# istellartech/GELATO

Hardware: AMD Instinct MI355X
Metric: residual+Jacobian evals/sec (and ms/eval), 6-phase x 64-node LGR mesh (higher is better)
Workload: dtype f64

## Files before the change

gelato_amd/csrc/gel_eval_kernel.h:

```cpp
#pragma once

namespace gel {

enum ParkSlot { PK_Q0 = 0, PK_Q1, PK_Q2, PK_Q3, PK_V0, PK_V1, PK_V2, PK_DJJ, PK_LV0, PK_LV1, PK_LV2,
                PK_FP0, PK_FP1, PK_FP2, PK_FP3, PK_FP4, PK_FP5, PK_FP6, PK_FP7, PK_COUNT };
constexpr int kStageLd = 17;
constexpr int kWaveLds = PK_COUNT * 64;
static_assert(kWaveLds >= 64 * kStageLd, "the MFMA staging tile must fit the wave's park region");
constexpr int kCoopStageOff = PK_LV0 * 64;
static_assert(kWaveLds - kCoopStageOff >= 64 * 11, "the cooperative hand-over area must fit behind the early park slots");
constexpr int kXldsPipeFrom = kLongPhaseFrom;
constexpr int kSlabRowsMax = 68, kPackRows = 36, kParkRes = (PK_LV2 + 1) * 64;
constexpr int kPipeSlabK = 8;
constexpr int wave_lds_doubles(bool jac, bool mfma, bool pack, bool split = false, bool longp = true) {
  return jac ? kWaveLds : (!mfma ? kParkRes : (split ? 64 * kStageLd  : (pack ? kParkRes + 4 * 64  : (longp ? 2 * 4 * kPipeSlabK * 11 + 64 * kPipeSlabK  : kSlabRowsMax * 11))));
}
static_assert(wave_lds_doubles(false, true, false, true) >= kParkRes, "residual-only split form: park over the result tile");
static_assert(wave_lds_doubles(false, true, true) >= 64 * 11 && wave_lds_doubles(false, true, false) >= 64 * 11 && wave_lds_doubles(false, true, false, false, false) >= 64 * 11, "hand-over area");
static_assert(wave_lds_doubles(false, true, true) >= kParkRes && wave_lds_doubles(false, true, false) >= kParkRes && wave_lds_doubles(false, true, false, false, false) >= kParkRes, "residual-only park");

constexpr int kSlotPT = 0, kSlotVM = 3, kSlotVP = 6;

#ifndef GEL_MIN_WAVES_PER_SIMD
#define GEL_MIN_WAVES_PER_SIMD 4
// ... 875 lines not shown
      PosCentreTail pt;
      double cen_rho = 0.0, cen_P = 0.0, cen_inv_a = 0.0;
      double dir2 = 0.0;
      EarthHalf aeh{1.0, 0.0};
      bool have_aeh = false;
#ifndef GEL_AEH
#define GEL_AEH aeh
#endif
#ifndef GEL_X_NOPOS
#define GEL_X_NOPOS 0
#endif
#ifndef GEL_X_NOQUAT
#define GEL_X_NOQUAT 0
#endif
#ifndef GEL_X_NOVEL
#define GEL_X_NOVEL 0
#endif
      const bool aero_on = AERO && akinds != 0;
      const bool a_need_alpha = AERO && (akinds & 5) != 0;
#define GEL_AERO_NEED_EA(ip_, wn_, we_)                                                                                \
  do {                                                                                                                 \
    if (!have_aeh && __builtin_amdgcn_ballot_w64(wind_needs_angle(ip_, wn_, we_)) != 0) {                               \
      int jl_ = jc;                                                                                                    \
      asm volatile("" : "+v"(jl_));    \
      const double tau_ = P.tau[ph.toff + jl_];                                                                        \
      const EarthAngle e_ = earth_angle((tau_ * (tf - to) / 2 + (tf + to) / 2) * P.ut);                                \
      aeh.ch = e_.ch; aeh.sh = e_.sh; have_aeh = true;                                                                 \
    }                                                                                                                  \
  } while (0)
#define GEL_AERO_FETCH()                                                                                               \
  const int ab_[3] = {load_const(&aph->base[0]), load_const(&aph->base[1]), load_const(&aph->base[2])};                \
  const double ax_[3] = {load_const(&aph->ilx[0]), load_const(&aph->ilx[1]), load_const(&aph->ilx[2])};                \
  const int n8_ = 8 * n, j08_ = 8 * j0
#define GEL_AERO_ENTRY(blk, col, a_, nv2_, d_, ind_, rho_, okl_, a_cc, a_ac, a_qc, a_isc, a_ok)                         \
  do {                                                                                                                 \
    double t_ = 0.0, dq_ = 0.0, qp_ = 0.0;                                                                             \
    const double ac_ = a_ac;                                                                                           \
    {                                                                                                                  \
      const double qc_ = a_qc;                                                                                         \
      qp_ = 0.5 * (rho_) * (nv2_);                                                                                     \
      dq_ = qp_ - qc_;                                                                                                 \
      if (a_need_alpha) {                                                                                              \
        const double cp_ = aero_cos(a_, nv2_, d_, ind_);                                                               \
        const bool okd_ = aero_dalpha(cp_, nv2_, a_cc, a_isc, a_ok, t_);                                               \
        if (__builtin_amdgcn_ballot_w64(!okd_) != 0) {                                                                 \
          const double t2_ = aero_acos(cp_, nv2_) - ac_;                                                               \
          t_ = okd_ ? t_ : t2_;                                                                                        \
        }                                                                                                              \
      }                                                                                                                \
    }                                                                                                                  \
    _Pragma("unroll") for (int kind = 0; kind < 3; kind++) {                                                           \
      if ((blk) == 2 && kind == 1) continue;                             \
      const double df_ = (kind == 0) ? t_ : ((kind == 1) ? dq_ : qp_ * t_ + dq_ * ac_);                                \
      const double gv = -(df_ * ax_[kind]);                                                                            \
      if (okl_) AEMIT(ab_[kind] + (((blk) == 0 ? 1 : ((blk) == 1 ? 4 : 7)) + (col)) * n8_ + j08_, gv);                 \
    }                                                                                                                  \
  } while (0)
#if GEL_CA_CACHE
      Bracket ca_br = no_bracket();
#define GEL_CA_BRACKET (JAC ? &ca_br : (Bracket*)nullptr)
#else
#define GEL_CA_BRACKET nullptr
#endif
      struct ParkSink { lds_double* park; GEL_DEV void put(int i, double v) const { if (!(AERO && (i == PCS_P || i == PCS_IH))) park[(PK_FP0 + i) * 64] = v; } };
      constexpr int PK_ACC = PK_FP0 + PCS_P, PK_AAC = PK_FP0 + PCS_IH, PK_AQC = PK_LV2;
      static_assert(PCS_COUNT == 8 && PK_FP7 == PK_FP0 + 7, "PosCentre's early members fill FP0-7");
      {
        PosPart pp;
        double v[3], w[3], F[3], dir[3];
        const double r[3] = {fresh_product(re[0], P.up), fresh_product(re[1], P.up), fresh_product(re[2], P.up)};
        if (JAC) pp = pos_part<true, ParkSink>(r, tb, P.barC20, nullptr, ParkSink{park}, &pt);
        else pp = pos_part(r, tb, P.barC20);
        const bool cen_windy = AERO && __builtin_amdgcn_ballot_w64(!(pp.wn == 0.0 && pp.we == 0.0)) != 0;
        if (__builtin_amdgcn_ballot_w64(wind_needs_angle(pp.inv_p, pp.wn, pp.we)) != 0) {
          const EarthAngle e0 = earth_angle(tn);
          eh.ch = e0.ch; eh.sh = e0.sh; have_eh = true;
          if (aero_on) PARK_SET(PK_ACC, tn);
        }
        EarthAngle ea{1.0, 0.0, 1.0, 0.0};
        if (have_eh) ea = full_angle(eh);
        wind_eci_or_calm(r, ea, pp.shp, pp.chp, pp.inv_p, pp.wn, pp.we, w);
#pragma unroll
        for (int c = 0; c < 3; c++) v[c] = PARK_GET(PK_V0 + c) * P.uv;
        aero_force(r, v, pp.rho, pp.inv_a, w, ph.area, tb, F, GEL_CA_BRACKET);
#define GEL_T (ph.thrust - ph.nozzle * pp.P)
#define GEL_TDC(name) const double name[3] = {GEL_T * dir[0], GEL_T * dir[1], GEL_T * dir[2]}
        {
          const double q[4] = {PARK_GET(PK_Q0), PARK_GET(PK_Q1), PARK_GET(PK_Q2), PARK_GET(PK_Q3)};
          thrust_dir(q, dir);
        }
        double tm[3];
        {
          GEL_TDC(Tdc);
          accel_parts(Tdc, F, inv_m, pp.g, inv_uv, tm, fc);
        }
        if (rb) {
#ifndef GEL_RES_XPOSE_VEL_AIR
#define GEL_RES_XPOSE_VEL_AIR 1
#endif
          if (!JAC || GEL_RES_XPOSE_VEL_AIR) {
            double cv[3];
#pragma unroll
            for (int c = 0; c < 3; c++) cv[c] = PARK_GET(PK_LV0 + c) - fc[c] * (tf - to) * hT;
            RSTORE_ROWS(wave_lds + PK_LV0 * 64, 3, rs_v, cv);
          } else {
#pragma unroll
            for (int c = 0; c < 3; c++) {
              const double cv = PARK_GET(PK_LV0 + c) - fc[c] * (tf - to) * hT;
              RSTORE(rs_v + 3 * gn + c, cv);
              GEL_CHK(cv);
            }
          }
        }
        if (JAC) {
          asm volatile("" ::: "memory");
          PARK_SET(PK_LV0, pp.shp); PARK_SET(PK_LV1, pp.chp);
          if (!AERO) PARK_SET(PK_LV2, pp.inv_p);
        }
        if (JAC && lead && !P.fd_recompute) GEL_MASS_CLOSED(tm);
        if (JAC && ph.air_fd && (SPLIT && P.split_vel ? !lead : lead)) {
          double f[3];
          {
            const double djj = PARK_GET(PK_DJJ);
#pragma unroll
            for (int k = 0; k < 3; k++) {
              if (SPLIT && P.split_vel && k != part - 1) continue;
              double vp[3], Fp[3];
#pragma unroll
              for (int c = 0; c < 3; c++) vp[c] = ((k == c) ? (PARK_GET(PK_V0 + c) + dx) : PARK_GET(PK_V0 + c)) * P.uv;
              const double r[3] = {fresh_product(re[0], P.up), fresh_product(re[1], P.up), fresh_product(re[2], P.up)};
              aero_force(r, vp, pp.rho, pp.inv_a, w, ph.area, tb, Fp, GEL_CA_BRACKET);
              GEL_TDC(Tdc);
              accel(Tdc, Fp, inv_m, pp.g, inv_uv, f);
#pragma unroll
              for (int c = 0; c < 3; c++) EMIT(ph.s_vv + 3 * k + c, ((c == k) ? djj : 0.0) + FDQ(f[c], fc[c]));
            }
          }
        }
        if (JAC && lead) {
          double f[3];
          if (!P.fd_recompute) {
            GEL_QUAT_CLOSED(GEL_T);
          } else if (P.fd_recompute) {
            const double q[4] = {PARK_GET(PK_Q0), PARK_GET(PK_Q1), PARK_GET(PK_Q2), PARK_GET(PK_Q3)};
#pragma unroll 1
            for (int k = 0; k < 4; k++) {
              double qp[4];
#pragma unroll
              for (int c = 0; c < 4; c++) qp[c] = (k == c) ? (q[c] + dx) : q[c];
              double dp[3];
              thrust_dir(qp, dp);
              const double Td[3] = {GEL_T * dp[0], GEL_T * dp[1], GEL_T * dp[2]};
              accel(Td, F, inv_m, pp.g, inv_uv, f);
#pragma unroll
              for (int c = 0; c < 3; c++) EMIT(ph.s_vq + 3 * k + c, FDQ(f[c], fc[c]));
            }
            GEL_TDC(Tdc);
            accel(Tdc, F, frcp((me + dx) * P.um), pp.g, inv_uv, f);
#pragma unroll
            for (int c = 0; c < 3; c++) EMIT(kSlotVM + c, FDQ(f[c], fc[c]));
          }
          if (!ph.t_fd) {
            const double vt[3] = {fc[0] * hT, fc[1] * hT, fc[2] * hT};
            EMIT_GROUP(3, ph.s_vt, vt, CG_VT, 0, true, true);
          }
        }
        if (aero_on) {
          asm volatile("" ::: "memory");
          const double ra[3] = {fresh_product(re[0], P.up), fresh_product(re[1], P.up), fresh_product(re[2], P.up)};
          double va[3], wa[3], a0[3];
#pragma unroll
          for (int c = 0; c < 3; c++) va[c] = PARK_GET(PK_V0 + c) * P.uv;
          if (have_eh) {
            const EarthAngle e1 = earth_angle(PARK_GET(PK_ACC) * P.ut);
            aeh.ch = e1.ch; aeh.sh = e1.sh; have_aeh = true;
          }
          if (cen_windy) {
            PosCentre pcx;
            double wn_, we_, p_, ip_, ih_;
            pos_centre_tail(pt, pp.rho, pp.P, tb, pcx, wn_, we_);
            geodetic_p_ih(ra[0], ra[1], ra[2], p_, ip_, ih_);
            EarthAngle e2{1.0, 0.0, 1.0, 0.0};
            if (have_aeh) e2 = full_angle(GEL_AEH);
            wind_eci(ra, e2, PARK_GET(PK_LV0), PARK_GET(PK_LV1), ip_, wn_, we_, wa);
          } else {
            wa[0] = 0.0; wa[1] = 0.0; wa[2] = 0.0;
          }
          const double nv2 = aero_vair2(ra, va, wa, a0);
          const double ind = frsqrt(fmax(dir[0] * dir[0] + dir[1] * dir[1] + dir[2] * dir[2], 1.0e-300));
          const double cc = a_need_alpha ? aero_cos(a0, nv2, dir, ind) : 0.0;
          const double alpha_c = a_need_alpha ? aero_acos(cc, nv2) : 0.0;
          const double qdyn_c = 0.5 * pp.rho * nv2;
          double sc, isc;
          fsqrt_rsqrt(fmax((1.0 - cc) * (1.0 + cc), 1.0e-300), sc, isc);
          const bool centre_ok = (cc <= 1.0) && (nv2 >= 1.0e-12) && (sc > 1.0e-6);
          GEL_AERO_FETCH();
          const double ail_[3] = {load_const(&aph->il[0]), load_const(&aph->il[1]), load_const(&aph->il[2])};
#pragma unroll
          for (int kind = 0; kind < 3; kind++) {
            const double il = ail_[kind];
            const double cv = 1.0 - ((kind == 0) ? alpha_c : (kind == 1) ? qdyn_c : qdyn_c * alpha_c) * il;
            AEMIT(ab_[kind] + j08_, cv);
            GEL_CHK(cv);
          }
          if (a_need_alpha && !GEL_X_NOQUAT) {
            const double q[4] = {PARK_GET(PK_Q0), PARK_GET(PK_Q1), PARK_GET(PK_Q2), PARK_GET(PK_Q3)};
#pragma unroll
            for (int c = 0; c < 4; c++) {
              double qp[4], dp[3];
#pragma unroll
              for (int d = 0; d < 4; d++) qp[d] = (d == c) ? q[d] + dx : q[d];
              thrust_dir(qp, dp);
              const double indp = frsqrt(fmax(dp[0] * dp[0] + dp[1] * dp[1] + dp[2] * dp[2], 1.0e-300));
              GEL_AERO_ENTRY(2, c, a0, nv2, dp, indp, pp.rho, true, cc, alpha_c, qdyn_c, isc, centre_ok);
              __builtin_amdgcn_sched_barrier(0);
            }
          }
#pragma unroll
          for (int c = 0; c < (GEL_X_NOVEL ? 0 : 3); c++) {
            double vp[3], a[3];
#pragma unroll
            for (int d = 0; d < 3; d++) vp[d] = ((d == c) ? PARK_GET(PK_V0 + d) + dx : PARK_GET(PK_V0 + d)) * P.uv;
            const double nv2p = aero_vair2(ra, vp, wa, a);
            GEL_AERO_ENTRY(1, c, a, nv2p, dir, ind, pp.rho, true, cc, alpha_c, qdyn_c, isc, centre_ok);
            __builtin_amdgcn_sched_barrier(0);
          }
          PARK_SET(PK_ACC, cc); PARK_SET(PK_AAC, centre_ok ? alpha_c : -alpha_c); PARK_SET(PK_AQC, qdyn_c);
        }
        if (JAC) {
          asm volatile("" ::: "memory");
          PARK_SET(PK_Q0, fc[0]); PARK_SET(PK_Q1, fc[1]); PARK_SET(PK_Q2, fc[2]); PARK_SET(PK_Q3, dir[0]); PARK_SET(PK_DJJ, dir[1]);
          dir2 = dir[2];
          cen_rho = pp.rho; cen_P = pp.P; cen_inv_a = pp.inv_a;
        }
#undef GEL_TDC
#undef GEL_T
      }
      if (JAC && (!SPLIT || part)) {
        const int k0 = SPLIT ? part - 1 : 0, k1 = SPLIT ? part : 3;
#define GEL_POS_SWEEP_F(rp, pq, f_)                                                                           \
  do {                                                                                                        \
    double wq_[3], Fp_[3];                                                                                    \
    GEL_NEED_EARTH_ANGLE((pq).inv_p, (pq).wn, (pq).we);                                                       \
    EarthAngle ea{1.0, 0.0, 1.0, 0.0};                                                                        \
    if (have_eh) ea = full_angle(eh);                                                                         \
    wind_eci_or_calm(rp, ea, (pq).shp, (pq).chp, (pq).inv_p, (pq).wn, (pq).we, wq_);                          \
    const double vq_[3] = {PARK_GET(PK_V0) * P.uv, PARK_GET(PK_V1) * P.uv, PARK_GET(PK_V2) * P.uv};           \
    aero_force(rp, vq_, (pq).rho, (pq).inv_a, wq_, ph.area, tb, Fp_, GEL_CA_BRACKET);                         \
    const double Tp_ = ph.thrust - ph.nozzle * (pq).P;                                                        \
// ... 247 lines not shown
```

gelato_amd/csrc/gel_host.hip:

```cpp
#include <hip/hip_runtime.h>

#include <algorithm>
#include <cmath>
#include <cstdio>
#include <chrono>
#include <atomic>
#include <cstdlib>
#include <cstring>
#include <memory>
#include <string>
#include <thread>
#include <vector>

#include "gel_host_handle.h"

namespace gelhost {
namespace {
thread_local std::string g_err;
}
int fail(int code, const std::string& msg) {
  g_err = msg;
  return code;
}
}
// ... 1256 lines not shown
  for (int k = 0; k < 3; k++) {
    const size_t n = p->aero.rows[k].size();
    off_c[k] = atotal; atotal += (io->aero_con[k] && n) ? n : 0;
    off_j[k] = atotal; atotal += (io->aero_con[k] && n && io->aero_jac[k]) ? aero_jac_len(p, k) : 0;
    aero = aero || (io->aero_con[k] && n);
  }
  const size_t nrows_out = rows ? R + 7 * nfn : 0;
  if (rows || aero) HIPCHK(p->h_arena.reserve(nrows_out + atotal));
  double* const h_rows = p->h_arena.get();
  double* const h_aero = h_rows + nrows_out;
  const bool x_pinned = p->cb_x[0].get() && (x == p->cb_x[0].get() || x == p->cb_x[1].get());
  if (!x_pinned) std::memcpy(p->h_x.get(), x, (size_t)p->dims.num_vars * 8);
  const double* const xin = x_pinned ? x : p->h_x.get();
  gel::ProblemDev dv = p->dev;
  dv.flag = p->h_flag.get();
  const bool want_jac = io->vals_full != nullptr;
  const bool fused = io->res || want_jac;
  static const int cb_mode = [] { const char* e = getenv("GEL_CB_MODE"); return e ? atoi(e) : 0; }();
  const bool split_exact = p->exact && want_jac;
  bool aero_jac = false;
  for (int k = 0; k < 3; k++) aero_jac = aero_jac || (io->aero_con[k] && io->aero_jac[k] && !p->aero.rows[k].empty());
  const bool split_aero = p->exact_aero && aero_jac;
  const bool split_rows = p->exact_rows && rows && io->rows_jfn;
  const bool coo = want_jac && cb_mode != 3 && !p->exact && !split_aero && !split_rows && coo_direct(p);
  if (coo) {
    if ((rc = ensure_full(p))) return rc;
    dv.coo_full = p->h_full.get(); dv.coo = p->d_coo.get();
  }
  dv.split_vel = 1;
  const bool own_res = io->res && p->cb_res.get() && io->res == p->cb_res.get();
  double* const res_to = own_res ? p->cb_res.get() : p->h_res.get();
  gel::AeroLaunchOut out;
  if (aero)
    for (int k = 0; k < 3; k++) {
      const size_t n = p->aero.rows[k].size();
      out.nrows[k] = (int32_t)n;
      out.con[k] = (io->aero_con[k] && n) ? h_aero + off_c[k] : nullptr;
      out.jac[k] = (out.con[k] && io->aero_jac[k]) ? h_aero + off_j[k] : nullptr;
    }
  if (cb_mode == 3 || !fused || split_exact || split_aero || split_rows) {
    if (fused) HIPCHK(launch_defects(p, dv, 1, xin, res_to, want_jac ? p->h_jv.get() : nullptr, p->stream.get()));
    if (rows) HIPCHK(launch_rows_kinds(p, dv, 1, xin, h_rows, io->rows_jfn ? h_rows + R : nullptr, p->stream.get()));
    if (aero) HIPCHK(launch_aero_kinds(p, dv, (int)p->aero.nodes.size(), p->aero.d_nodes.get(), 1, xin, out, p->stream.get()));
  } else {
    arm_done(p, dv);
    HIPCHK(gel::launch_callback(dv, want_jac, xin, res_to, want_jac ? p->h_jv.get() : nullptr,
                                aero ? (int)p->aero.nodes.size() : 0, p->aero.d_nodes.get(), aero ? &out : nullptr,
                                (int)nlin, p->d_lin_rows.get(), (int)nfn, p->d_fn_rows.get(), rows ? h_rows : nullptr,
                                (rows && io->rows_jfn) ? h_rows + R : nullptr, p->stream.get()));
  }
  HIPCHK(wait_done(p, dv));
  if (io->res && !own_res) std::memcpy(io->res, p->h_res.get(), (size_t)11 * p->dims.N * 8);
  if (want_jac) {
    if (coo) finish_full(p, io->vals_full, io->fill_constants);
    else scatter_full(p, p->h_jv.get(), io->vals_full, io->fill_constants);
  }
  if (rows) {
    std::memcpy(io->rows_con, h_rows, R * 8);
    if (io->rows_jfn) std::memcpy(io->rows_jfn, h_rows + R, 7 * nfn * 8);
  }
  if (aero)
    for (int k = 0; k < 3; k++) {
      if (out.con[k]) std::memcpy(io->aero_con[k], out.con[k], p->aero.rows[k].size() * 8);
      if (out.jac[k]) std::memcpy(io->aero_jac[k], out.jac[k], aero_jac_len(p, k) * 8);
    }
  if (*p->h_flag.get()) { *p->h_flag.get() = 0; return GEL_NONFINITE; }
  return GEL_OK;
}

int gel_table_limits(int32_t wind_rows, int32_t ca_rows, int32_t n, int64_t* info) {
  if (wind_rows < 2 || ca_rows < 2 || !info) return fail(GEL_ERR_ARG, "bad argument");
  const size_t T = gel::staged_table_doubles(wind_rows, ca_rows), Tp = gel::padded_table_doubles(wind_rows, ca_rows);
  info[0] = (int64_t)T;
  info[1] = (int64_t)lds_room(gel::eval_lds_bytes_max(wind_rows, ca_rows) / 8 - Tp, true);
  info[2] = (int64_t)lds_room(gel::aero_lds_bytes(wind_rows, ca_rows) / 8 - Tp, true);
  info[3] = (n >= 2 && n < gel::kMeshMaxThreads) ? (int64_t)lds_room(gel::mesh_vector_doubles(n), true) : -1;
  info[4] = (int64_t)lds_room(gel::table_lds_bytes(wind_rows, ca_rows) / 8 - T, false);
  info[5] = (int64_t)gel::kLaunchMaxLds;
  info[6] = info[3] < 0 ? -1 : (int64_t)gel::mesh_vectors_per_group(wind_rows, ca_rows, n);
  return GEL_OK;
}

int gel_point_eval(int32_t kind, int32_t n, const double* in, const double* aux, int32_t aux_rows, double* out) {
  static const int nin[16] = {1, 3, 3, 6, 7, 1, 1, 2, 2, 8, 8, 8, 7, 4, 1, 5}, nout[16] = {5, 3, 3, 3, 3, 3, 1, 4, 6, 8, 16, 4, 3, 7, 2, 18};
  if (kind < 0 || kind > 15 || n < 0 || !in || !out) return fail(GEL_ERR_ARG, "bad argument");
  if (n == 0) return GEL_OK;
  const bool tabulated = kind == 5 || kind == 6 || kind == 9 || kind == 10 || kind == 15;
  int rc = tabulated ? check_launch_lds("gel_point_eval", gel::point_lds_bytes(aux_rows), 5 * (size_t)std::max(aux_rows, 0), 5 * (size_t)std::max(aux_rows, 0), false) : GEL_OK;
  if (rc) return rc;
  rc = need_device();
  if (rc) return rc;
  double atm[gel::kAtmTableDoubles];
  size_t naux = 0;
  const double* hax = aux;
  std::vector<double> ext;
  if (kind == 0) { gel::fill_atmosphere_table(atm); hax = atm; naux = gel::kAtmTableDoubles; aux_rows = 0; }
  else if (kind == 2) { if (!aux) return fail(GEL_ERR_ARG, "kind 2 needs aux[0] = barC20"); naux = 1; aux_rows = 0; }
  else if (tabulated) {
    const int w = (kind == 5 || kind == 10 || kind == 15) ? 3 : 2;
    if (!aux || aux_rows < 2) return fail(GEL_ERR_ARG, "kinds 5, 6, 9, 10 and 15 need a table of at least two rows");
    if (kind == 15) { gel::fill_atmosphere_table(atm); ext.assign(atm, atm + gel::kAtmTableDoubles); }
    for (int k = 1; k < aux_rows; k++)
      if (!(aux[(size_t)w * k] > aux[(size_t)w * (k - 1)])) return fail(GEL_ERR_ARG, "table abscissae must increase strictly");
    std::vector<double> slopes;
    gel::append_rows_and_slopes(ext, slopes, aux, aux_rows, w);
    ext.insert(ext.end(), slopes.begin(), slopes.end());
    hax = ext.data(); naux = ext.size();
  }
  else { aux_rows = 0; }
  DeviceArray<double> i, a, o;
  HIPCHK(i.upload(in, (size_t)n * nin[kind])); HIPCHK(a.upload(hax, naux)); HIPCHK(o.reserve((size_t)n * nout[kind]));
  HIPCHK(gel::launch_point(kind, n, i.get(), a.get(), aux_rows, o.get(), nullptr));
  HIPCHK(hipMemcpy(out, o.get(), (size_t)n * nout[kind] * 8, hipMemcpyDeviceToHost));
  return GEL_OK;
}

}
```

gelato_amd/csrc/gel_kernels.hip:

```cpp
#include <hip/hip_runtime.h>

#include "gel_tables.h"
#include "gel_output_row.h"

#include "gel_eval_kernel.h"
namespace gel {

constexpr int kExpandGroup = 8;
__global__ __launch_bounds__(kBlock) void expand_kernel(long long nnz, long long V, int B, const double* __restrict__ cval,
                                                        const int32_t* __restrict__ src,
                                                        const double* __restrict__ jvar, double* __restrict__ full) {
  const int b0 = blockIdx.y * kExpandGroup;
  const int nb = min(kExpandGroup, B - b0);
  const bool even = (nnz & 1) == 0;
  for (long long i = 2 * ((long long)blockIdx.x * kBlock + threadIdx.x); i < nnz; i += 2LL * gridDim.x * kBlock) {
    const bool two = i + 1 < nnz;
    const int s0 = src[i], s1 = two ? src[i + 1] : -1;
    const double c0 = (s0 == -1) ? cval[i] : 0.0, c1 = (two && s1 == -1) ? cval[i + 1] : 0.0;
    const int g0 = (s0 >= 0) ? s0 : -2 - s0, g1 = (s1 >= 0) ? s1 : -2 - s1;
    for (int g = 0; g < nb; g++) {
      const double* jv = jvar + (size_t)(b0 + g) * V;
      double* out = full + (size_t)(b0 + g) * nnz + i;
      const double v0 = (s0 == -1) ? c0 : ((s0 >= 0) ? jv[g0] : -jv[g0]);
      const double v1 = (s1 == -1) ? c1 : ((s1 >= 0) ? jv[g1] : -jv[g1]);
// ... 43 lines not shown
}

__global__ void perturb_local_kernel(int nloc, double dx, const double* __restrict__ x, const int32_t* __restrict__ colmap,
                                     double* __restrict__ Xp) {
  const long long t = (long long)blockIdx.x * blockDim.x + threadIdx.x;
  if (t >= (long long)(nloc + 1) * nloc) return;
  const int row = (int)(t / nloc), col = (int)(t - (long long)row * nloc);
  double v = x[colmap[col]];
  if (row == col + 1) v += dx;
  Xp[t] = v;
}

__global__ void quotient_local_kernel(int nloc, int nres, int roff, int nrows, double dx, const double* __restrict__ res,
                                      double* __restrict__ J, long long ldJ, int row0, const int32_t* __restrict__ colmap) {
  __shared__ double tile[32][33];
  const int c0 = blockIdx.x * 32, r0 = blockIdx.y * 32;
  for (int k = threadIdx.y; k < 32; k += blockDim.y) {
    const int c = c0 + k, r = r0 + threadIdx.x;
    if (c < nloc && r < nrows) tile[k][threadIdx.x] = res[(size_t)(c + 1) * nres + roff + r];
  }
  __syncthreads();
  for (int k = threadIdx.y; k < 32; k += blockDim.y) {
    const int r = r0 + k, c = c0 + threadIdx.x;
    if (c < nloc && r < nrows) J[(size_t)(row0 + r) * ldJ + (colmap ? colmap[c] : c)] = (tile[threadIdx.x][k] - res[roff + r]) / dx;
  }
}

struct RhsArgs {
  int n, Kw, Kc;
  const double *mass_e, *pos_e, *vel_e, *quat, *t, *tables;
  double thrust, area, nozzle, um, up, uv, barC20;
  double* out;
};

__global__ void rhs_vel_air_kernel(RhsArgs A) {
  extern __shared__ double lds[];
  ProblemDev P{};
  P.Kw = A.Kw; P.Kc = A.Kc; P.tables = A.tables;
  const Tables tb = stage_tables(P, lds);
  const int i = blockIdx.x * blockDim.x + threadIdx.x;
  if (i >= A.n) return;
  const double m = A.mass_e[i] * A.um;
  const double r[3] = {A.pos_e[3 * i] * A.up, A.pos_e[3 * i + 1] * A.up, A.pos_e[3 * i + 2] * A.up};
  const double v[3] = {A.vel_e[3 * i] * A.uv, A.vel_e[3 * i + 1] * A.uv, A.vel_e[3 * i + 2] * A.uv};
  const double q[4] = {A.quat[4 * i], A.quat[4 * i + 1], A.quat[4 * i + 2], A.quat[4 * i + 3]};
  const PosPart pp = pos_part(r, tb, A.barC20);
  const EarthAngle ea = earth_angle(A.t[i]);
  double w[3], F[3], dir[3], f[3];
  wind_eci(r, ea, pp.shp, pp.chp, pp.inv_p, pp.wn, pp.we, w);
  aero_force(r, v, pp.rho, pp.inv_a, w, A.area, tb, F);
  thrust_dir(q, dir);
  const double T = A.thrust - A.nozzle * pp.P;
  const double Td[3] = {T * dir[0], T * dir[1], T * dir[2]};
  accel(Td, F, 1.0 / m, pp.g, 1.0 / A.uv, f);
  for (int c = 0; c < 3; c++) A.out[3 * i + c] = f[c];
}

__global__ void rhs_vel_noair_kernel(RhsArgs A) {
  const int i = blockIdx.x * blockDim.x + threadIdx.x;
  if (i >= A.n) return;
  const double m = A.mass_e[i] * A.um;
  const double r[3] = {A.pos_e[3 * i] * A.up, A.pos_e[3 * i + 1] * A.up, A.pos_e[3 * i + 2] * A.up};
  const double q[4] = {A.quat[4 * i], A.quat[4 * i + 1], A.quat[4 * i + 2], A.quat[4 * i + 3]};
  double dir[3], g[3], f[3];
  thrust_dir(q, dir);
  gravity_eci(r, A.barC20, g);
  const double Td[3] = {A.thrust * dir[0], A.thrust * dir[1], A.thrust * dir[2]};
  accel_noair(Td, 1.0 / m, g, 1.0 / A.uv, f);
  for (int c = 0; c < 3; c++) A.out[3 * i + c] = f[c];
}

__global__ void rhs_quat_kernel(int n, const double* quat, const double* u_e, double unit_u, double* out) {
  const int i = blockIdx.x * blockDim.x + threadIdx.x;
  if (i >= n) return;
  const double q[4] = {quat[4 * i], quat[4 * i + 1], quat[4 * i + 2], quat[4 * i + 3]};
  double dq[4];
  quat_rate(q, u_e[2 * i], u_e[2 * i + 1], unit_u, dq);
  for (int c = 0; c < 4; c++) out[4 * i + c] = dq[c];
}

__global__ void point_kernel(int kind, int n, const double* in, const double* aux, int aux_rows, double* out) {
  extern __shared__ double lds[];
  const int naux = (kind == 5 || kind == 10) ? 3 * aux_rows + 2 * (aux_rows - 1)
                   : (kind == 6 || kind == 9) ? 2 * aux_rows + (aux_rows - 1)
                   : (kind == 15) ? kAtmDoubles + 3 * aux_rows + 2 * (aux_rows - 1) : (kind == 0 ? kAtmDoubles : 0);
  for (int i = threadIdx.x; i < naux; i += blockDim.x) lds[i] = aux[i];
  __syncthreads();
  const int i = blockIdx.x * blockDim.x + threadIdx.x;
  if (i >= n) return;
  switch (kind) {
    case 0: {
      const double h = geopotential_altitude(in[i]);
      const Air a = atmosphere(h, lds);
      out[5 * i] = h; out[5 * i + 1] = a.T; out[5 * i + 2] = a.P; out[5 * i + 3] = a.rho; out[5 * i + 4] = a.a;
    } break;
    case 1: {
      double lat, sl, cl, p, ip;
      geodetic_lat_p(in[3 * i], in[3 * i + 1], in[3 * i + 2], lat, p, ip);
      geodetic_sincos_p(in[3 * i], in[3 * i + 1], in[3 * i + 2], sl, cl, p, ip);
      const double lon = atan2(in[3 * i + 1], in[3 * i]);
      out[3 * i] = lat * 180.0 / kPi; out[3 * i + 1] = lon * 180.0 / kPi;
      out[3 * i + 2] = geodetic_alt_from(p, sl, cl);
    } break;
    case 2: {
      const double r[3] = {in[3 * i], in[3 * i + 1], in[3 * i + 2]};
      double g[3];
      gravity_eci(r, aux[0], g);
      out[3 * i] = g[0]; out[3 * i + 1] = g[1]; out[3 * i + 2] = g[2];
    } break;
    case 3: {
      const double* a = in + 6 * i;
      const double r[3] = {a[0], a[1], a[2]};
      double sl, cl, p, ip, w[3];
      geodetic_sincos_p(r[0], r[1], r[2], sl, cl, p, ip);
      const EarthAngle ea = earth_angle(a[3]);
      double chp, irt;
      fsqrt_rsqrt(0.5 * (1.0 + cl), chp, irt);
      wind_eci(r, ea, (0.5 * sl) * irt, chp, ip, a[4], a[5], w);
      out[3 * i] = w[0]; out[3 * i + 1] = w[1]; out[3 * i + 2] = w[2];
    } break;
    case 4: {
      const double* a = in + 7 * i;
      double s, c;
      sincos(kOmega * a[6], &s, &c);
      const double d0 = a[0] - (0.0 * a[5] - kOmega * a[4]);
      const double d1 = a[1] - (kOmega * a[3] - 0.0 * a[5]);
      const double d2 = a[2] - (0.0 * a[4] - 0.0 * a[3]);
      out[3 * i] = d0 * c + d1 * s; out[3 * i + 1] = -d0 * s + d1 * c; out[3 * i + 2] = d2;
    } break;
    case 5: {
      double wn, we;
      wind_ned2(in[i], lds, lds + 3 * aux_rows, aux_rows, wn, we);
      out[3 * i] = wn; out[3 * i + 1] = we; out[3 * i + 2] = 0.0;
    } break;
    case 6: out[i] = interp_tab(in[i], lds, lds + 2 * aux_rows, aux_rows, 2, 1); break;
    case 7: {
      const double a = in[2 * i], b = in[2 * i + 1];
      out[4 * i] = fsqrt(a); out[4 * i + 1] = sqrt(a); out[4 * i + 2] = fdiv(a, b); out[4 * i + 3] = a / b;
    } break;
    case 8: {
      double s1, c1, s2, c2;
      fsincos(in[2 * i], &s1, &c1);
      sincos(in[2 * i], &s2, &c2);
      out[6 * i] = s1; out[6 * i + 1] = c1; out[6 * i + 2] = s2; out[6 * i + 3] = c2;
      out[6 * i + 4] = flog_ratio(in[2 * i + 1]); out[6 * i + 5] = log(in[2 * i + 1]);
    } break;
    case 9: {
      Bracket br = no_bracket();
      for (int k = 0; k < 8; k++) out[8 * i + k] = interp_tab_cached(in[8 * i + k], lds, lds + 2 * aux_rows, aux_rows, 2, 1, br);
    } break;
    case 10: {
      Bracket2 br = no_bracket2();
      for (int k = 0; k < 8; k++) {
        double wn, we;
        wind_ned2_cached(in[8 * i + k], lds, lds + 3 * aux_rows, aux_rows, wn, we, br);
        out[16 * i + 2 * k] = wn; out[16 * i + 2 * k + 1] = we;
      }
    } break;
    case 11: {
      double o[4];
      quatmult(in + 8 * i, in + 8 * i + 4, o);
      for (int c = 0; c < 4; c++) out[4 * i + c] = o[c];
    } break;
    case 12: {
      double o[3];
      quatrot(in + 7 * i, in + 7 * i + 4, o);
      for (int c = 0; c < 3; c++) out[3 * i + c] = o[c];
    } break;
    case 13: {
      const double* q = in + 4 * i;
      out[7 * i] = q[0]; out[7 * i + 1] = -q[1]; out[7 * i + 2] = -q[2]; out[7 * i + 3] = -q[3];
      double d[3];
      thrust_dir(q, d);
      for (int c = 0; c < 3; c++) out[7 * i + 4 + c] = d[c];
    } break;
    case 14: out[2 * i] = fexp(in[i]); out[2 * i + 1] = exp(in[i]); break;
    case 15: {
      Tables tb;
      tb.atm = lds; tb.wind = lds + kAtmDoubles; tb.winds = tb.wind + 3 * aux_rows; tb.ca = nullptr; tb.cas = nullptr;
      tb.Kw = aux_rows; tb.Kc = 0;
      const double* a = in + 5 * i;
      const double r[3] = {a[0], a[1], a[2]};
      const int kk = min(max((int)a[3], 0), 2);
      PosCentre pc;
      PosCentreTail pt;
      PosPart pp = pos_part<true, PosCentreSink, false>(r, tb, 0.0, nullptr, PosCentreSink{&pc}, &pt);
      pos_centre_tail(pt, pp.rho, pp.P, tb, pc, pp.wn, pp.we);
      PosPart pq;
      const bool ok = pos_delta(r, kk, a[4], pp, pc, tb, pq);
      double* o = out + 18 * i;
      o[0] = pp.rho; o[1] = pp.P; o[2] = pp.inv_a; o[3] = pp.wn; o[4] = pp.we; o[5] = pp.shp; o[6] = pp.chp; o[7] = pp.inv_p;
      o[8] = pq.rho; o[9] = pq.P; o[10] = pq.inv_a; o[11] = pq.wn; o[12] = pq.we; o[13] = pq.shp; o[14] = pq.chp; o[15] = pq.inv_p;
      o[16] = ok ? 1.0 : 0.0; o[17] = pc.margin;
    } break;
    default: break;
  }
}

struct AeroPos {
  double rho;
  double wn, we;
  double shp, chp, inv_p;
};

GEL_DEV AeroPos aero_pos_part(const double r[3], const Tables& tb) {
  AeroPos o;
  double lat, p, sl, cl;
  geodetic_lat_p(r[0], r[1], r[2], lat, p, o.inv_p);
  fsincos(lat, &sl, &cl);
  const double h = geopotential_altitude(geodetic_alt_from(p, sl, cl));
  wind_ned2(h, tb.wind, tb.winds, tb.Kw, o.wn, o.we);
  double irt;
  fsqrt_rsqrt(0.5 * (1.0 + cl), o.chp, irt);
  o.shp = (0.5 * sl) * irt;
  o.rho = atmosphere(h, tb.atm).rho;
  return o;
}

GEL_DEV double aero_vair(const double r[3], const double v[3], const EarthAngle& ea, const double w[3], double a[3]) {
  const double d0 = v[0] + kOmega * r[1], d1 = v[1] - kOmega * r[0];
  const double e0 = d0 * ea.c + d1 * ea.s, e1 = -d0 * ea.s + d1 * ea.c;
  a[0] = (e0 * ea.c - e1 * ea.s) - w[0]; a[1] = (e0 * ea.s + e1 * ea.c) - w[1]; a[2] = v[2] - w[2];
  return sqrt(a[0] * a[0] + a[1] * a[1] + a[2] * a[2]);
}

GEL_DEV double aero_alpha(const double a[3], double nv, const double q[4]) {
  double dir[3];
  thrust_dir(q, dir);
  const double nd = sqrt(dir[0] * dir[0] + dir[1] * dir[1] + dir[2] * dir[2]);
  const double c_alpha = (a[0] / nv) * (dir[0] / nd) + (a[1] / nv) * (dir[1] / nd) + (a[2] / nv) * (dir[2] / nd);
  return (c_alpha > 1.0) ? 0.0 : ((nv < 1e-6) ? 0.0 : acos(c_alpha));
}

struct AeroOut {
  double* con[3];
  double* jac[3];
  int32_t nrows[3];
  int64_t ld;
  int32_t sm;
};

#ifndef GEL_AERO_UNROLL
#define GEL_AERO_UNROLL 1
#endif
constexpr int kAeroWaves = 4;
enum { AP_ILIM = 0, AP_AC = 3, AP_QC, AP_CC, AP_IS, AP_IND, AP_W = 8, AP_A0 = 11, AP_DIR = 14, AP_RHO = 17, AP_NV2 = 18, AP_INTS = 19,
       kAeroParkSlots = 25 };
static_assert(wave_lds_doubles(false, false, false) <= kWaveLds && wave_lds_doubles(false, true, false, true) <= kWaveLds &&
              wave_lds_doubles(false, true, true) <= kWaveLds && wave_lds_doubles(false, true, false, false, true) <= kWaveLds &&
              wave_lds_doubles(false, true, false, false, false) <= kWaveLds, "kWaveLds is the largest region");
static size_t eval_lds_bytes(size_t park_off, int wave_doubles) { return sizeof(double) * (park_off + (size_t)wave_doubles * (kBlock / 64)); }
size_t eval_lds_bytes_max(int Kw, int Kc) { return eval_lds_bytes(padded_table_doubles(Kw, Kc), kWaveLds); }
size_t aero_lds_bytes(int Kw, int Kc) { return sizeof(double) * (padded_table_doubles(Kw, Kc) + (size_t)kAeroWaves * kAeroParkSlots * 64); }
typedef __attribute__((address_space(3))) int lds_int;
typedef __attribute__((address_space(3))) double lds_f64;
template <bool ROLES, bool WIDE = false, bool SM = false>
__device__ __forceinline__ void aero_body(const ProblemDev P, int nnodes, const AeroNodeDev* __restrict__ nodes, int tiles, int B,
                                          const double* __restrict__ x, const AeroOut O, const unsigned vblk) {
  extern __shared__ double lds[];
  const Tables tb = stage_tables(P, lds);
  const int lane = (int)(threadIdx.x & 63);
  const int sw = ROLES ? (int)(threadIdx.x >> 6) : -1;
  const long long wid = ROLES ? (long long)vblk : (long long)vblk * kAeroWaves + __builtin_amdgcn_readfirstlane((int)(threadIdx.x >> 6));
  const bool flat = !ROLES && !WIDE && tiles == 0;
  int b, ni_raw;
  bool live;
  if (WIDE) {
    const long long total = (long long)B * nnodes, f = wid * 64 + lane;
    if (wid * 64 >= total) return;
    live = f < total;
    const long long fc = live ? f : total - 1;
    b = (int)(fc / nnodes);
    ni_raw = live ? (int)(fc - (long long)b * nnodes) : nnodes;
  } else if (flat) {
    const long long total = (long long)B * nnodes, f0 = wid * 64;
    if (f0 >= total) return;
// ... 656 lines not shown
```

gelato_amd/csrc/gel_rhs_parts.h:

```cpp
#pragma once
#include "gel_physics.h"

#ifndef GEL_CALM_SHORTCUT
#define GEL_CALM_SHORTCUT 1
#endif

namespace gel {

struct PosPart {
  double rho, P, inv_a;
  double wn, we;
  double g[3];
  double shp, chp;
  double inv_p;
};

GEL_DEV void geodetic_sincos(double x, double y, double z, double& sl, double& cl, double& p) {
  p = sqrt(x * x + y * y);
  const double a = z * kRa, b = p * kRb;
  const double ih = 1.0 / sqrt(a * a + b * b);
  const double st = a * ih, ct = b * ih;
  const double zz = z + kEp2 * kRb * (st * st * st);
  const double pp = p - kE2 * kRa * (ct * ct * ct);
  const double ihy = 1.0 / sqrt(zz * zz + pp * pp);
// ... 134 lines not shown
}
GEL_DEV EarthAngle earth_angle(double t) {
  EarthAngle e;
  fsincos(kOmega * t / 2.0, &e.sh, &e.ch);
  e.s = 2.0 * e.sh * e.ch;
  e.c = (e.ch - e.sh) * (e.ch + e.sh);
  return e;
}

#ifndef GEL_WIND_CHAIN
#define GEL_WIND_CHAIN 0
#endif
GEL_DEV bool wind_needs_angle(double inv_p, double wn, double we) {
  const bool windy = !(wn == 0.0 && we == 0.0);
#if GEL_WIND_CHAIN
  return windy;
#else
  return windy && !(inv_p > 0.0);
#endif
}
GEL_DEV void wind_eci_chain(const double r[3], const EarthAngle& e, double s_hp, double c_hp, double inv_p, double wn,
                            double we, double w[3]) {
  const double px = r[0] * e.c + r[1] * e.s;
  const double py = -r[0] * e.s + r[1] * e.c;
  const double clon = (inv_p > 0.0) ? px * inv_p : 1.0, slon = py * inv_p;
  double th, ith;
  fsqrt_rsqrt(0.5 * (1.0 + fabs(clon)), th, ith);
  const double uh = (0.5 * slon) * ith;
  const double c_hl = (clon >= 0.0) ? th : fabs(uh);
  const double s_hl = (clon >= 0.0) ? uh : copysign(th, slon);
  const double irt2 = 0.70710678118654752440;
  const double b0 = c_hl * (c_hp - s_hp) * irt2, b1 = s_hl * (c_hp + s_hp) * irt2;
  const double b2 = -c_hl * (c_hp + s_hp) * irt2, b3 = s_hl * (c_hp - s_hp) * irt2;
  const double q0 = e.ch * b0 - e.sh * b3;
  const double q1 = -(e.ch * b1 - e.sh * b2);
  const double q2 = -(e.ch * b2 + e.sh * b1);
  const double q3 = -(e.ch * b3 + e.sh * b0);
  const double t0 = -wn * q1 - we * q2;
  const double t1 = wn * q0 + we * q3;
  const double t2 = -wn * q3 + we * q0;
  const double t3 = wn * q2 - we * q1;
  w[0] = q0 * t1 - q1 * t0 - q2 * t3 + q3 * t2;
  w[1] = q0 * t2 + q1 * t3 - q2 * t0 - q3 * t1;
  w[2] = q0 * t3 - q1 * t2 + q2 * t1 - q3 * t0;
}
GEL_DEV void wind_eci(const double r[3], const EarthAngle& e, double s_hp, double c_hp, double inv_p, double wn,
                      double we, double w[3]) {
#if GEL_WIND_CHAIN
  wind_eci_chain(r, e, s_hp, c_hp, inv_p, wn, we, w);
#else
  const bool off_axis = inv_p > 0.0;
  const double clon = off_axis ? r[0] * inv_p : e.c;
  const double slon = off_axis ? r[1] * inv_p : e.s;
  const double sl = fresh_mul(2.0 * s_hp, c_hp);
  const double cl = fresh_mul(c_hp - s_hp, c_hp + s_hp);
  const double nh = -fresh_mul(wn, sl);
  w[0] = __builtin_fma(nh, clon, -fresh_mul(we, slon));
  w[1] = __builtin_fma(nh, slon, fresh_mul(we, clon));
  w[2] = fresh_mul(wn, cl);
#endif
}

GEL_DEV void wind_eci_or_calm(const double r[3], const EarthAngle& e, double s_hp, double c_hp, double inv_p, double wn,
                              double we, double w[3]) {
#if GEL_CALM_SHORTCUT
  if (__builtin_amdgcn_ballot_w64(!(wn == 0.0 && we == 0.0)) == 0) {
    w[0] = 0.0; w[1] = 0.0; w[2] = 0.0;
    return;
  }
#endif
  wind_eci(r, e, s_hp, c_hp, inv_p, wn, we, w);
}
GEL_DEV void wind_eci_chain_or_calm(const double r[3], const EarthAngle& e, double s_hp, double c_hp, double inv_p, double wn,
                                    double we, double w[3]) {
#if GEL_CALM_SHORTCUT
  if (__builtin_amdgcn_ballot_w64(!(wn == 0.0 && we == 0.0)) == 0) {
    w[0] = 0.0; w[1] = 0.0; w[2] = 0.0;
    return;
  }
#endif
  wind_eci_chain(r, e, s_hp, c_hp, inv_p, wn, we, w);
}

GEL_DEV void aero_force(const double r[3], const double v[3], double rho, double inv_a_sound, const double w[3], double area,
                        const Tables& tb, double F[3], Bracket* br = nullptr) {
  const double d0 = v[0] + kOmega * r[1];
  const double d1 = v[1] - kOmega * r[0];
  const double a0 = d0 - w[0];
  const double a1 = d1 - w[1];
  const double a2 = v[2] - w[2];
  const double vn = fsqrt(fmax(a0 * a0 + a1 * a1 + a2 * a2, 1.0e-200));
  const double mach = vn * inv_a_sound;
  const double ca = br ? interp_tab_cached(mach, tb.ca, tb.cas, tb.Kc, 2, 1, *br) : interp_tab(mach, tb.ca, tb.cas, tb.Kc, 2, 1);
  const double k = 0.5 * rho * area * ca * vn;
  F[0] = k * -a0; F[1] = k * -a1; F[2] = k * -a2;
}

GEL_DEV void accel(const double Td[3], const double F[3], double inv_m, const double g[3], double inv_uv,
                   double out[3]) {
#pragma unroll
  for (int c = 0; c < 3; c++) out[c] = ((Td[c] + F[c]) * inv_m + g[c]) * inv_uv;
}
GEL_DEV void accel_parts(const double Td[3], const double F[3], double inv_m, const double g[3], double inv_uv, double tm[3],
                         double out[3]) {
#pragma unroll
  for (int c = 0; c < 3; c++) { tm[c] = (Td[c] + F[c]) * inv_m; out[c] = (tm[c] + g[c]) * inv_uv; }
}
GEL_DEV void accel_noair(const double Td[3], double inv_m, const double g[3], double inv_uv, double out[3]) {
#pragma unroll
  for (int c = 0; c < 3; c++) out[c] = (Td[c] * inv_m + g[c]) * inv_uv;
}

GEL_DEV void thrust_dir(const double q[4], double dir[3]) {
  dir[0] = q[0] * q[0] + q[1] * q[1] - q[2] * q[2] - q[3] * q[3];
  dir[1] = q[0] * q[3] + q[1] * q[2] + q[2] * q[1] + q[3] * q[0];
  dir[2] = -q[0] * q[2] + q[1] * q[3] - q[2] * q[0] + q[3] * q[1];
}

GEL_DEV void quat_rate(const double q[4], double u0, double u1, double unit_u, double dq[4]) {
  const double d2r = 0.017453292519943295769;
  const double oy = (u0 * unit_u) * d2r, oz = (u1 * unit_u) * d2r;
  dq[0] = 0.5 * (-q[2] * oy - q[3] * oz);
  dq[1] = 0.5 * (q[2] * oz - q[3] * oy);
  dq[2] = 0.5 * (q[0] * oy - q[1] * oz);
  dq[3] = 0.5 * (q[0] * oz + q[1] * oy);
}

GEL_DEV double aero_vair2(const double r[3], const double v[3], const double w[3], double a[3]) {
  a[0] = (v[0] + kOmega * r[1]) - w[0]; a[1] = (v[1] - kOmega * r[0]) - w[1]; a[2] = v[2] - w[2];
  return a[0] * a[0] + a[1] * a[1] + a[2] * a[2];
}
GEL_DEV double aero_cos(const double a[3], double nv2, const double d[3], double ind) {
  return ((a[0] * d[0] + a[1] * d[1] + a[2] * d[2]) * frsqrt(fmax(nv2, 1.0e-300))) * ind;
}
GEL_DEV double aero_acos(double c, double nv2) { return (c > 1.0) ? 0.0 : ((nv2 < 1.0e-12) ? 0.0 : acos(c)); }
GEL_DEV bool aero_dalpha(double c_p, double nv2_p, double c_c, double inv_s, bool centre_ok, double& t) {
  const double t0 = (c_c - c_p) * inv_s, k = (0.5 * c_c) * inv_s;
  const double t1 = t0 - (k * t0) * t0;
  t = (t0 - (k * t1) * t1) + (t1 * t1) * (t1 * (1.0 / 6.0));
  return centre_ok && (c_p <= 1.0) && (nv2_p >= 1.0e-12) && (fabs(k * t0) < 1.0e-4);
}


}
```

gelato_amd/dynamics.py:

```python
import ctypes as C

import numpy as np

from ._lib import check, lib

_dp = C.POINTER(C.c_double)


def _f(a):
    return np.ascontiguousarray(a, dtype=np.float64)


def _d(a):
    return a.ctypes.data_as(_dp)


def dynamics_velocity(mass_e, pos_eci_e, vel_eci_e, quat_eci2body, t, param, wind_table, CA_table, units, barC20=0.0):
    mass_e, pos, vel, quat, t = _f(mass_e), _f(pos_eci_e), _f(vel_eci_e), _f(quat_eci2body), _f(t)
    param, wind, ca, units = _f(param), _f(wind_table), _f(CA_table), _f(units)
    n = mass_e.shape[0]
    if pos.shape != (n, 3) or vel.shape != (n, 3) or quat.shape != (n, 4) or t.shape != (n,):
        raise TypeError("dynamics_velocity(): incompatible function arguments (shape mismatch)")
    out = np.zeros((n, 3))
    check(lib().gel_dynamics_velocity(n, _d(mass_e), _d(pos), _d(vel), _d(quat), _d(t), _d(param), _d(wind),
                                      wind.shape[0], _d(ca), ca.shape[0], _d(units), float(barC20), _d(out)))
    return out


def dynamics_velocity_NoAir(mass_e, pos_eci_e, quat_eci2body, param, units, barC20=0.0):
    mass_e, pos, quat, param, units = _f(mass_e), _f(pos_eci_e), _f(quat_eci2body), _f(param), _f(units)
    n = mass_e.shape[0]
    if pos.shape != (n, 3) or quat.shape != (n, 4):
        raise TypeError("dynamics_velocity_NoAir(): incompatible function arguments (shape mismatch)")
    out = np.zeros((n, 3))
    check(lib().gel_dynamics_velocity_NoAir(n, _d(mass_e), _d(pos), _d(quat), _d(param), _d(units), float(barC20),
                                            _d(out)))
    return out


def dynamics_quaternion(quat_eci2body, u_e, unit_u):
    quat, u = _f(quat_eci2body), _f(u_e)
    n = quat.shape[0]
    if quat.shape != (n, 4) or u.shape != (n, 2):
        raise TypeError("dynamics_quaternion(): incompatible function arguments (shape mismatch)")
    out = np.zeros((n, 4))
    check(lib().gel_dynamics_quaternion(n, _d(quat), _d(u), float(unit_u), _d(out)))
    return out


def point_eval(kind, x, aux=None):
    nin = [1, 3, 3, 6, 7, 1, 1, 2, 2, 8, 8, 8, 7, 4, 1, 5][kind]
    nout = [5, 3, 3, 3, 3, 3, 1, 4, 6, 8, 16, 4, 3, 7, 2, 18][kind]
    x = _f(x).reshape(-1, nin)
    n = x.shape[0]
    out = np.zeros((n, nout))
    a = _f(aux) if aux is not None else None
    rows = 0 if a is None else (a.shape[0] if a.ndim == 2 else 0)
    check(lib().gel_point_eval(kind, n, _d(x), _d(a) if a is not None else None, rows, _d(out)))
    return out
```

Baseline: 23.09 million.

## Replace velocity finite-difference drag recomputation with an analytic drag delta

The velocity Jacobian entries no longer rerun the full aero_force for each perturbed velocity component. aero_force now records a DragCentre (relative airspeed, norm, reciprocal norm, CA slope and Mach bracket), and drag_delta evaluates the perturbed drag from a series expansion of the norm plus the linear CA segment. Lanes where the expansion or bracket check fails fall back to the old finite-difference path in a deferred pass. A new point_eval kind exposes drag_delta for testing. The cost is extra state per lane, ballot-driven divergence, and a fallback loop that still calls aero_force twice per component.

Measured after the change: 22.93 million. Within noise of the previous version (-0.7%).

```diff
diff --git a/gelato_amd/csrc/gel_eval_kernel.h b/gelato_amd/csrc/gel_eval_kernel.h
--- a/gelato_amd/csrc/gel_eval_kernel.h
+++ b/gelato_amd/csrc/gel_eval_kernel.h
@@ -981,7 +981,35 @@
         wind_eci_or_calm(r, ea, pp.shp, pp.chp, pp.inv_p, pp.wn, pp.we, w);
 #pragma unroll
         for (int c = 0; c < 3; c++) v[c] = PARK_GET(PK_V0 + c) * P.uv;
-        aero_force(r, v, pp.rho, pp.inv_a, w, ph.area, tb, F, GEL_CA_BRACKET);
+        const bool vel_mine = JAC && ph.air_fd && (SPLIT && P.split_vel ? !lead : lead);
+        unsigned todo_v = 0;
+        DragCentre dc;
+        aero_force(r, v, pp.rho, pp.inv_a, w, ph.area, tb, F, GEL_CA_BRACKET, JAC ? &dc : (DragCentre*)nullptr);
+        if (vel_mine && P.fd_recompute) {
+          todo_v = (SPLIT && P.split_vel) ? 1u << (part - 1) : 7u;
+        } else if (vel_mine) {
+          const double djj = PARK_GET(PK_DJJ);
+          const double kv = (inv_m * inv_uv) * fds;
+          dc.Kca = dc.Kca * -kv; dc.Ksia = dc.Ksia * -kv;
+#pragma unroll
+          for (int k = 0; k < 3; k++) {
+            if (SPLIT && P.split_vel && k != part - 1) continue;
+            const double vk = PARK_GET(PK_V0 + k);
+            const double vk0 = vk * P.uv;
+            const double vk1 = (vk + dx) * P.uv;
+            const double dl = vk1 - vk0;
+            double dF[3];
+            const bool ok = drag_delta(dc, k, dl, dF);
+            if (__builtin_amdgcn_ballot_w64(!ok) != 0) {
+              todo_v |= 1u << k;
+              if (__builtin_amdgcn_ballot_w64(ok) == 0) continue;
+            }
+            if (ok) {
+#pragma unroll
+              for (int c = 0; c < 3; c++) EMIT(ph.s_vv + 3 * k + c, (c == k) ? djj + dF[c] : dF[c]);
+            }
+          }
+        }
 #define GEL_T (ph.thrust - ph.nozzle * pp.P)
 #define GEL_TDC(name) const double name[3] = {GEL_T * dir[0], GEL_T * dir[1], GEL_T * dir[2]}
         {
@@ -1017,25 +1045,40 @@
           if (!AERO) PARK_SET(PK_LV2, pp.inv_p);
         }
         if (JAC && lead && !P.fd_recompute) GEL_MASS_CLOSED(tm);
-        if (JAC && ph.air_fd && (SPLIT && P.split_vel ? !lead : lead)) {
-          double f[3];
-          {
-            const double djj = PARK_GET(PK_DJJ);
-#pragma unroll
-            for (int k = 0; k < 3; k++) {
-              if (SPLIT && P.split_vel && k != part - 1) continue;
-              double vp[3], Fp[3];
-#pragma unroll
-              for (int c = 0; c < 3; c++) vp[c] = ((k == c) ? (PARK_GET(PK_V0 + c) + dx) : PARK_GET(PK_V0 + c)) * P.uv;
-              const double r[3] = {fresh_product(re[0], P.up), fresh_product(re[1], P.up), fresh_product(re[2], P.up)};
-              aero_force(r, vp, pp.rho, pp.inv_a, w, ph.area, tb, Fp, GEL_CA_BRACKET);
-              GEL_TDC(Tdc);
-              accel(Tdc, Fp, inv_m, pp.g, inv_uv, f);
-#pragma unroll
-              for (int c = 0; c < 3; c++) EMIT(ph.s_vv + 3 * k + c, ((c == k) ? djj : 0.0) + FDQ(f[c], fc[c]));
-            }
-          }
-        }
+        constexpr bool kVelTodoLate = !PACK && !AERO;
+#define GEL_VEL_TODO_PASS()                                                                                                             \
+        if (todo_v) {                                                                                                                   \
+          const double djj = PARK_GET(PK_DJJ);                                                                                          \
+          _Pragma("unroll 1")                                                                                                           \
+          for (int k = 0; k < 3; k++) {                                                                                                 \
+            if (!((todo_v >> k) & 1u)) continue;                                                                      \
+            const double r[3] = {fresh_product(re[0], P.up), fresh_product(re[1], P.up), fresh_product(re[2], P.up)};                   \
+            double vp[3], Fp[3], f[3];                                                                                                  \
+            bool ok = false;               \
+            if (!P.fd_recompute) {                                                                                                      \
+              const double vc[3] = {PARK_GET(PK_V0) * P.uv, PARK_GET(PK_V1) * P.uv, PARK_GET(PK_V2) * P.uv};                            \
+              DragCentre dc2;                                                                                                           \
+              aero_force(r, vc, pp.rho, pp.inv_a, w, ph.area, tb, Fp, GEL_CA_BRACKET, &dc2);                                            \
+              const double vk = PARK_GET(PK_V0 + k);                                                                                    \
+              const double vk0 = vk * P.uv;                                                                                             \
+              const double vk1 = (vk + dx) * P.uv;                                                                                      \
+              const double dl = vk1 - vk0;                                                                                              \
+              ok = drag_delta(dc2, k, dl, f);                                                                                           \
+            }                                                                                                                           \
+            __builtin_amdgcn_sched_barrier(0);     \
+            _Pragma("unroll")                                                                                                           \
+            for (int c = 0; c < 3; c++) vp[c] = ((k == c) ? (PARK_GET(PK_V0 + c) + dx) : PARK_GET(PK_V0 + c)) * P.uv;                   \
+            aero_force(r, vp, pp.rho, pp.inv_a, w, ph.area, tb, Fp, GEL_CA_BRACKET);                                                    \
+            GEL_TDC(Tdc);                                                                                                               \
+            accel(Tdc, Fp, inv_m, pp.g, inv_uv, f);                                                                                     \
+                                        \
+            if (!ok) {                                                                                                                  \
+            _Pragma("unroll")                                                                                                           \
+              for (int c = 0; c < 3; c++) EMIT(ph.s_vv + 3 * k + c, ((c == k) ? djj : 0.0) + FDQ(f[c], fc[c]));                         \
+            }                                                                                                                           \
+          }                                                                                                                             \
+        }
+        if (!kVelTodoLate) GEL_VEL_TODO_PASS();
         if (JAC && lead) {
           double f[3];
           if (!P.fd_recompute) {
@@ -1064,6 +1107,8 @@
             EMIT_GROUP(3, ph.s_vt, vt, CG_VT, 0, true, true);
           }
         }
+        if (kVelTodoLate) GEL_VEL_TODO_PASS();
+#undef GEL_VEL_TODO_PASS
         if (aero_on) {
           asm volatile("" ::: "memory");
           const double ra[3] = {fresh_product(re[0], P.up), fresh_product(re[1], P.up), fresh_product(re[2], P.up)};
diff --git a/gelato_amd/csrc/gel_host.hip b/gelato_amd/csrc/gel_host.hip
--- a/gelato_amd/csrc/gel_host.hip
+++ b/gelato_amd/csrc/gel_host.hip
@@ -1362,10 +1362,10 @@
 }
 
 int gel_point_eval(int32_t kind, int32_t n, const double* in, const double* aux, int32_t aux_rows, double* out) {
-  static const int nin[16] = {1, 3, 3, 6, 7, 1, 1, 2, 2, 8, 8, 8, 7, 4, 1, 5}, nout[16] = {5, 3, 3, 3, 3, 3, 1, 4, 6, 8, 16, 4, 3, 7, 2, 18};
-  if (kind < 0 || kind > 15 || n < 0 || !in || !out) return fail(GEL_ERR_ARG, "bad argument");
+  static const int nin[17] = {1, 3, 3, 6, 7, 1, 1, 2, 2, 8, 8, 8, 7, 4, 1, 5, 14}, nout[17] = {5, 3, 3, 3, 3, 3, 1, 4, 6, 8, 16, 4, 3, 7, 2, 18, 4};
+  if (kind < 0 || kind > 16 || n < 0 || !in || !out) return fail(GEL_ERR_ARG, "bad argument");
   if (n == 0) return GEL_OK;
-  const bool tabulated = kind == 5 || kind == 6 || kind == 9 || kind == 10 || kind == 15;
+  const bool tabulated = kind == 5 || kind == 6 || kind == 9 || kind == 10 || kind == 15 || kind == 16;
   int rc = tabulated ? check_launch_lds("gel_point_eval", gel::point_lds_bytes(aux_rows), 5 * (size_t)std::max(aux_rows, 0), 5 * (size_t)std::max(aux_rows, 0), false) : GEL_OK;
   if (rc) return rc;
   rc = need_device();
@@ -1378,7 +1378,7 @@
   else if (kind == 2) { if (!aux) return fail(GEL_ERR_ARG, "kind 2 needs aux[0] = barC20"); naux = 1; aux_rows = 0; }
   else if (tabulated) {
     const int w = (kind == 5 || kind == 10 || kind == 15) ? 3 : 2;
-    if (!aux || aux_rows < 2) return fail(GEL_ERR_ARG, "kinds 5, 6, 9, 10 and 15 need a table of at least two rows");
+    if (!aux || aux_rows < 2) return fail(GEL_ERR_ARG, "kinds 5, 6, 9, 10, 15 and 16 need a table of at least two rows");
     if (kind == 15) { gel::fill_atmosphere_table(atm); ext.assign(atm, atm + gel::kAtmTableDoubles); }
     for (int k = 1; k < aux_rows; k++)
       if (!(aux[(size_t)w * k] > aux[(size_t)w * (k - 1)])) return fail(GEL_ERR_ARG, "table abscissae must increase strictly");
diff --git a/gelato_amd/csrc/gel_kernels.hip b/gelato_amd/csrc/gel_kernels.hip
--- a/gelato_amd/csrc/gel_kernels.hip
+++ b/gelato_amd/csrc/gel_kernels.hip
@@ -149,7 +149,7 @@
 __global__ void point_kernel(int kind, int n, const double* in, const double* aux, int aux_rows, double* out) {
   extern __shared__ double lds[];
   const int naux = (kind == 5 || kind == 10) ? 3 * aux_rows + 2 * (aux_rows - 1)
-                   : (kind == 6 || kind == 9) ? 2 * aux_rows + (aux_rows - 1)
+                   : (kind == 6 || kind == 9 || kind == 16) ? 2 * aux_rows + (aux_rows - 1)
                    : (kind == 15) ? kAtmDoubles + 3 * aux_rows + 2 * (aux_rows - 1) : (kind == 0 ? kAtmDoubles : 0);
   for (int i = threadIdx.x; i < naux; i += blockDim.x) lds[i] = aux[i];
   __syncthreads();
@@ -259,6 +259,20 @@
       o[0] = pp.rho; o[1] = pp.P; o[2] = pp.inv_a; o[3] = pp.wn; o[4] = pp.we; o[5] = pp.shp; o[6] = pp.chp; o[7] = pp.inv_p;
       o[8] = pq.rho; o[9] = pq.P; o[10] = pq.inv_a; o[11] = pq.wn; o[12] = pq.we; o[13] = pq.shp; o[14] = pq.chp; o[15] = pq.inv_p;
       o[16] = ok ? 1.0 : 0.0; o[17] = pc.margin;
+    } break;
+    case 16: {
+      Tables tb;
+      tb.atm = nullptr; tb.wind = nullptr; tb.winds = nullptr; tb.ca = lds; tb.cas = lds + 2 * aux_rows;
+      tb.Kw = 0; tb.Kc = aux_rows;
+      const double* a = in + 14 * i;
+      const double r[3] = {a[0], a[1], a[2]}, v[3] = {a[3], a[4], a[5]}, w[3] = {a[6], a[7], a[8]};
+      const int k = min(max((int)a[12], 0), 2);
+      DragCentre dc;
+      double F[3], dF[3];
+      aero_force(r, v, a[9], a[10], w, a[11], tb, F, nullptr, &dc);
+      const bool ok = drag_delta(dc, k, a[13], dF);
+      double* o = out + 4 * i;
+      o[0] = dF[0]; o[1] = dF[1]; o[2] = dF[2]; o[3] = ok ? 1.0 : 0.0;
     } break;
     default: break;
   }
diff --git a/gelato_amd/csrc/gel_rhs_parts.h b/gelato_amd/csrc/gel_rhs_parts.h
--- a/gelato_amd/csrc/gel_rhs_parts.h
+++ b/gelato_amd/csrc/gel_rhs_parts.h
@@ -240,18 +240,60 @@
   wind_eci_chain(r, e, s_hp, c_hp, inv_p, wn, we, w);
 }
 
+struct DragCentre {
+  double a[3];
+  double vn, ivn;
+  double Kca;
+  double Ksia;
+  double inv_a;
+  double mlo, mhi;
+};
 GEL_DEV void aero_force(const double r[3], const double v[3], double rho, double inv_a_sound, const double w[3], double area,
-                        const Tables& tb, double F[3], Bracket* br = nullptr) {
+                        const Tables& tb, double F[3], Bracket* br = nullptr, DragCentre* dc = nullptr) {
   const double d0 = v[0] + kOmega * r[1];
   const double d1 = v[1] - kOmega * r[0];
   const double a0 = d0 - w[0];
   const double a1 = d1 - w[1];
   const double a2 = v[2] - w[2];
-  const double vn = fsqrt(fmax(a0 * a0 + a1 * a1 + a2 * a2, 1.0e-200));
+  const double n2 = a0 * a0 + a1 * a1 + a2 * a2;
+  double vn, ivn;
+  fsqrt_rsqrt(fmax(n2, 1.0e-200), vn, ivn);
   const double mach = vn * inv_a_sound;
   const double ca = br ? interp_tab_cached(mach, tb.ca, tb.cas, tb.Kc, 2, 1, *br) : interp_tab(mach, tb.ca, tb.cas, tb.Kc, 2, 1);
-  const double k = 0.5 * rho * area * ca * vn;
+  const double K = 0.5 * rho * area;
+  const double k = K * ca * vn;
   F[0] = k * -a0; F[1] = k * -a1; F[2] = k * -a2;
+  if (dc) {
+    const int n = tb.Kc;
+    const int idx = br ? br->idx : min(max(lower_count(mach, tb.ca, n, 2) - 1, 0), n - 2);
+    const double x0 = tb.ca[0], xn = tb.ca[2 * (n - 1)];
+    const bool below = mach <= x0, above = mach > xn;
+    dc->a[0] = a0; dc->a[1] = a1; dc->a[2] = a2;
+    dc->vn = vn; dc->ivn = ivn; dc->inv_a = inv_a_sound;
+    dc->Kca = K * ca;
+    dc->Ksia = (below || above) ? 0.0 : K * (tb.cas[idx] * inv_a_sound);
+    const double inf = __builtin_inf();
+    dc->mlo = !(n2 > 1.0e-200) ? inf : (below ? -inf : (above ? xn : tb.ca[2 * idx]));
+    dc->mhi = below ? x0 : (above ? inf : tb.ca[2 * idx + 2]);
+  }
+}
+
+GEL_DEV bool drag_delta(const DragCentre& c, int k, double dl, double dF[3]) {
+  const double ak = (k == 0) ? c.a[0] : ((k == 1) ? c.a[1] : c.a[2]);
+  const double q = dl * __builtin_fma(2.0, ak, dl);
+  const double u = q * c.ivn * c.ivn;
+  const double ser = __builtin_fma(u, __builtin_fma(u, 0.0625, -0.125), 0.5);
+  const double dvn = (c.vn * u) * ser;
+  const double vn1 = c.vn + dvn;
+  const double m1 = vn1 * c.inv_a;
+  const double Kds = dvn * __builtin_fma(c.Ksia, vn1, c.Kca);
+  const double Ks1 = __builtin_fma(c.Kca, c.vn, Kds);
+#pragma unroll
+  for (int i = 0; i < 3; i++) {
+    const double t = Kds * c.a[i];
+    dF[i] = -((i == k) ? __builtin_fma(Ks1, dl, t) : t);
+  }
+  return (fabs(u) < 1.0e-4) && (c.mlo < m1) && (m1 <= c.mhi);
 }
 
 GEL_DEV void accel(const double Td[3], const double F[3], double inv_m, const double g[3], double inv_uv,
diff --git a/gelato_amd/dynamics.py b/gelato_amd/dynamics.py
--- a/gelato_amd/dynamics.py
+++ b/gelato_amd/dynamics.py
@@ -49,8 +49,8 @@
 
 
 def point_eval(kind, x, aux=None):
-    nin = [1, 3, 3, 6, 7, 1, 1, 2, 2, 8, 8, 8, 7, 4, 1, 5][kind]
-    nout = [5, 3, 3, 3, 3, 3, 1, 4, 6, 8, 16, 4, 3, 7, 2, 18][kind]
+    nin = [1, 3, 3, 6, 7, 1, 1, 2, 2, 8, 8, 8, 7, 4, 1, 5, 14][kind]
+    nout = [5, 3, 3, 3, 3, 3, 1, 4, 6, 8, 16, 4, 3, 7, 2, 18, 4][kind]
     x = _f(x).reshape(-1, nin)
     n = x.shape[0]
     out = np.zeros((n, nout))
```
